# SYSTRAN/faster-whisper

Hardware: AMD Instinct MI355X
Metric: audio-sec/sec (RTF) large-v3 fp16 beam=5 batch=16 (higher is better)
Workload: dtype f16

## Files before the change

### faster_whisper_amd/_lib.py

```python
import ctypes as C
import os

import numpy as np

_HERE = os.path.dirname(os.path.abspath(__file__))
LIB_PATH = os.environ.get("FWAMD_LIB") or os.path.join(_HERE, "libfwamd.so")

FW_OK = 0
FW_EINVAL = -1
FW_ENODEV = -2
FW_ENOMEM = -3
FW_ERUNTIME = -4
FW_ENOSPC = -5

COMPUTE_FLOAT16 = 0
COMPUTE_INT8_FLOAT16 = 1
FW_DT_F32 = 0
FW_DT_F16 = 1
FW_MAX_ALIGN_HEADS = 64


class FwConfig(C.Structure):
    _fields_ = [
        ("n_mels", C.c_int32), ("n_audio_ctx", C.c_int32), ("d_model", C.c_int32), ("n_heads", C.c_int32),
# ... 40 lines not shown
    "fw_model_set_merge_wait", "fw_model_set_decode_lanes", "fw_model_run_capacity", "fw_dec_big_min_rows", "fw_dec_big_min_rows_of", "fw_test_knob",
    "fw_test_idle_lead_chunks",
    "fw_pack_blob_size", "fw_pack_blob_copy", "fw_pack_blob_free",
    "fw_logmel", "fw_logmel_full",
    "fw_encode", "fw_encode_pcm", "fw_encode_pcm_dev", "fw_tensor_shape", "fw_tensor_to_host",
    "fw_tensor_from_host", "fw_tensor_free",
    "fw_generate", "fw_generate_lp", "fw_detect_language", "fw_align",
    "fw_prof_enable", "fw_prof_reset", "fw_prof_count", "fw_prof_name", "fw_prof_get", "fw_synchronize",
    "fw_dev_alloc", "fw_dev_free", "fw_dev_upload",
    "fw_test_gemm", "fw_test_layernorm", "fw_test_attention", "fw_test_dec_linear", "fw_test_dec_logits", "fw_test_logits_rules",
    "fw_test_dec_self_attn", "fw_test_dec_cross_attn", "fw_test_dec_cross_probs", "fw_test_dec_softmax_pick", "fw_bench_gemm", "fw_bench_dec_linear", "fw_bench_attention",
    "fw_bench_gemm_epi", "fw_bench_dec_linear_epi",
    "fw_test_gemm_ex", "fw_test_cross_kv_frag_index", "fw_test_quant_rows", "fw_test_layernorm_frag",
    "fw_test_dec_beam_update", "fw_test_dec_embed", "fw_test_align_post",
    "fw_test_logits_rules_lp", "fw_test_dec_beam_update_lp",
    "fw_vad_create", "fw_vad_forward", "fw_vad_free", "fw_vad_forward_dev", "fw_vad_forward_audio_dev",
    "fw_vad_forward_audio_batch_dev",
    "fw_flac_info", "fw_flac_decode",
    "fw_resample_filter", "fw_resample_dev", "fw_bench_resample",
]

_lib = None


class FwError(RuntimeError):
    pass


def load():
    global _lib
# ... 70 lines not shown
    lib.fw_test_gemm.argtypes = [vp, vp, vp, vp, vp, i32, i32, i32, i32, i32, vp]
    lib.fw_test_dec_linear.argtypes = [vp, vp, vp, vp, vp, vp, vp, i32, i32, i32, i32, i32, vp, vp]
    lib.fw_test_dec_logits.argtypes = [vp, vp, i32, vp]
    lib.fw_test_logits_rules.argtypes = [vp, vp, i32, vp, i32, vp, C.POINTER(FwGenOpts), i32, vp, vp]
    if hasattr(lib, "fw_test_dec_self_attn"):
        lib.fw_test_dec_self_attn.argtypes = [vp, vp, vp, vp, vp, i32, i32, i32, i32, i32, i32, i32, i32, i32, i32, i32, vp]
        lib.fw_test_dec_cross_attn.argtypes = [vp, vp, vp, vp, i32, i32, i32, i32, i32, i32, vp, vp, i32, C.c_float, vp]
        lib.fw_test_dec_cross_probs.argtypes = [vp, vp, vp, i32, i32, i32, vp, i32, i32, i32, i32, vp]
        lib.fw_test_dec_softmax_pick.argtypes = [vp, vp, i32, i32, i32, vp, i32, vp]
    lib.fw_bench_attention.argtypes = [vp, i32, i32, i32, i32, i32, f32p]
    lib.fw_bench_gemm.argtypes = [vp, i32, i32, i32, i32, i32, i32, i32, i32, f32p]
    lib.fw_bench_dec_linear.argtypes = [vp, i32, i32, i32, i32, i32, i32, f32p]
    if hasattr(lib, "fw_bench_gemm_epi"):
        lib.fw_bench_gemm_epi.argtypes = [vp, i32, i32, i32, i32, i32, i32, i32, i32, i32, i32, i32, f32p]
        lib.fw_bench_dec_linear_epi.argtypes = [vp, i32, i32, i32, i32, i32, i32, i32, i32, i32, f32p]
    lib.fw_test_layernorm.argtypes = [vp, vp, vp, vp, i32, i32, vp]
    lib.fw_test_attention.argtypes = [vp, vp, vp, vp, i32, i32, i32, vp]
    if hasattr(lib, "fw_test_gemm_ex"):
        lib.fw_test_gemm_ex.argtypes = [vp, vp, i64, i64, i64, vp, vp, vp, i64, i64, i64, vp, i64, i64, i64, i64, i64,
                                        i32, i32, i32, i32, i32, i32, i32, i32, i32, vp, vp]
        lib.fw_test_cross_kv_frag_index.argtypes = [i32, i32, i32, vp]
        lib.fw_test_quant_rows.argtypes = [vp, vp, i32, i32, i64, vp, vp, i32, vp, vp]
        lib.fw_test_layernorm_frag.argtypes = [vp, vp, vp, vp, i32, i32, i32, vp]
    if hasattr(lib, "fw_test_dec_beam_update"):
        f32 = C.c_float
        lib.fw_test_dec_beam_update.argtypes = [vp, i32, i32, i32, i32, i32, i32, i32, i32, f32, i32, vp, vp, vp, vp, vp,
                                                i32, f32, vp, vp, vp, vp, vp, vp, vp, vp, vp, vp, vp]
        lib.fw_test_dec_embed.argtypes = [vp, vp, i32, vp, i32, vp, i32, i32, i32, i32, i32, i32, f32, vp, vp]
        lib.fw_test_align_post.argtypes = [vp, vp, i32, i32, i32, i32, vp, vp, i32, vp]
    if hasattr(lib, "fw_test_dec_beam_update_lp"):
# ... 46 lines not shown
```

### faster_whisper_amd/csrc/dec_kernels.h

```cpp
#pragma once
#include "common.h"

namespace fwd {

constexpr int FIN_CAP = 48;

struct GenDev {
  int B, K, R;
  int P;
  int budget;
  int max_fin;
  int V, n_text_ctx;
  int with_ts, suppress_blank, min_new, mits, ngram;
  float rep_pen, lp_pow;
  int eot, no_ts, ts_begin;
  int n_sup_begin, sup_begin[8];
  int sample;
  float inv_temp;
  unsigned seed_lo, seed_hi;
  int kv_div;
  int ctx, cache_rows;
  int ragged, reach;
};

// ... 22 lines not shown
                           int N, int K, int act);
int launch_dec_gemm_skinny_tiles(hipStream_t st, int tiles, const half_t* xf, const half_t* Wf, const half_t* bias,
                                 const float* s1, const float* cf, const half_t* res, int ldr, half_t* out, int ldo,
                                 half_t* out_frag, int R, int N, int K, int act);
int launch_dec_gemm_big(hipStream_t st, int cfg, const half_t* xf, const half_t* Wf, const half_t* bias, const float* s1,
                        const float* cf, const half_t* res, int ldr, half_t* out, int ldo, half_t* out_frag, int R,
                        int N, int K, int act);
int launch_dec_gemm_frag_variant(hipStream_t st, int variant, bool lnf, const half_t* xf, const half_t* Wf,
                                 const half_t* bias, const float* s1, const float* cf, half_t* out, int R, int N,
                                 int K);
int launch_dec_gemm_frag_i8(hipStream_t st, const int8_t* xq, const float* x_scale, const int8_t* Wq,
                            const float* w_scale, const half_t* bias, const half_t* res, int ldr, half_t* out, int ldo,
                            int R, int N, int K, int act);
int launch_dec_logits(hipStream_t st, bool i8, const void* xf, const float* x_scale, const void* Wf,
                      const float* w_scale, const float* s1, const float* cf, float* out, int ldo, int R, int N, int K);
void launch_nospeech(hipStream_t st, const float* logits, int V, int row_mul, int no_speech_id, float* out, int B);
#define LP_SUP_WORDS 896
void launch_logits_process(hipStream_t st, const GenDev& gp, float* logits, const unsigned long long* sup_bits,
                           const int* hist2, const float* cum2, const int* d_step, const int* done, float* cand_val,
                           int* cand_tok, float* cand_lp = nullptr);
void launch_beam_update(hipStream_t st, const GenDev& gp, const float* cand_val, const int* cand_tok, int* hist2,
                        float* cum2, uint8_t* kvidx2, int* cur_tok, const int* d_step, int* done, int* n_done,
                        int* n_fin, int* fin_tok, int* fin_len, float* fin_score, float* fin_cum,
                        const float* cand_lp = nullptr, float* lphist2 = nullptr, float* fin_lp = nullptr,
                        const int* ptab = nullptr);
void launch_gather_sot_rows(hipStream_t st, const half_t* x, const int* sot_tab, const int* ptab, int pos0, int nb,
                            int rows_per_chunk, half_t* xo, half_t* xof, int d, int B);
void launch_step_advance(hipStream_t st, int* d_step);
void launch_token_prob(hipStream_t st, const float* logits, int V, const int* target, float* out, int out_stride,
                       int out_off, int rows, int row_mul = 1);
// ... 5 lines not shown
```

### faster_whisper_amd/csrc/dec_kernels.hip

```cpp
#include "common.h"
#include "dec_kernels.h"
#include <stdlib.h>
#include <atomic>
#include <type_traits>

namespace fwd {
static std::atomic<int> g_self_attn_form{0};
static std::atomic<int> g_forms_epoch{0};
static std::atomic<int> g_cross_regs{0};
}

__device__ __forceinline__ size_t frag_off(int row, int k, int KS) {
  return ((size_t)((row >> 4) * KS + (k >> 5)) * 64 + ((k >> 3) & 3) * 16 + (row & 15)) * 8 + (k & 7);
}

static __device__ __forceinline__ int ragged_pos(const int* __restrict__ ptab, int chunk, int step, int reach) {
  const int p = ptab[chunk] - 1 + step;
  return p < reach ? p : reach - 1;
}

__global__ void dec_embed_kernel(const int* __restrict__ tok, const half_t* __restrict__ emb,
                                 const half_t* __restrict__ pos_emb, half_t* __restrict__ x,
                                 half_t* __restrict__ xfrag, int d, const int* __restrict__ d_step, int pos_fixed,
                                 int P, int blk_n, const int* __restrict__ ptab, int kmul, int reach) {
// ... 52 lines not shown
      const float t = tv - mu * a4[e];
      tv = rstd * t + c4[e];
    } else if (bias) {
      tv = tv + (float)b4[e];
    }
    if (act == 1) {
      const float er = erff(tv * 0.70710678118654752440f);
      tv = (0.5f * tv) * (1.0f + er);
    }
    if (has_res) tv = tv + (float)r4[e];
    o[e] = (half_t)tv;
  }
  return o;
}

static __device__ __forceinline__ half4_t dec_epilogue4_i8(const int (&v)[4], float sx, const float* __restrict__ w_scale,
                                                           const half_t* __restrict__ bias, const half_t* __restrict__ res,
                                                           int ldr, int row, int n, int act) {
#pragma clang fp contract(off)
  const floatx4 w4 = *reinterpret_cast<const floatx4*>(w_scale + n);
  half4_t b4 = {(half_t)0.f, (half_t)0.f, (half_t)0.f, (half_t)0.f}, r4 = b4;
  if (bias) b4 = *reinterpret_cast<const half4_t*>(bias + n);
  if (res) r4 = *reinterpret_cast<const half4_t*>(res + (size_t)row * ldr + n);
  half4_t o;
#pragma unroll
  for (int e = 0; e < 4; ++e) {
    float tv = ((float)v[e] * sx) * w4[e];
    if (bias) tv = tv + (float)b4[e];
    if (act == 1) {
      const float er = erff(tv * 0.70710678118654752440f);
// ... 160 lines not shown
#define DGB_TL_DECL
#endif
template <int N_>
static __device__ __forceinline__ void wait_vmcnt() {
  asm volatile("s_waitcnt vmcnt(%0)" ::"n"(N_) : "memory");
}
#define DGB_BARRIER()                      \
  do {                                     \
    asm volatile("" ::: "memory");         \
    __builtin_amdgcn_s_barrier();          \
    asm volatile("" ::: "memory");         \
  } while (0)

#define DGB_BARRIER_LDS() __syncthreads()

template <bool LNF, int S, int WM, int WN, int FB, int KC, int NST>
__global__ __launch_bounds__(WM * WN * 64, 2) void dec_gemm_big_kernel(
    const half_t* __restrict__ xf, const half_t* __restrict__ Wf, const half_t* __restrict__ bias,
    const float* __restrict__ s1, const float* __restrict__ cf, const half_t* __restrict__ res, int ldr,
    half_t* __restrict__ out, int ldo, half_t* __restrict__ out_frag, int R, int N, int K, int act, int nNt) {
  constexpr int NW = WM * WN;
  DGB_TL_DECL;
  constexpr int PX = 4 * WM, PW = FB * WN, PCS = PX + PW;
  static_assert((PCS * KC) % NW == 0, "pieces of a stage must divide over the waves");
  static_assert(FB == 2 || FB == 4, "column tiles per wave");
  constexpr int PPW = PCS * KC / NW;
  constexpr int STAGE_BYTES = PCS * KC * 1024;
  static_assert(NST >= 3 && NST <= 6, "ring depth");
  constexpr int DGB_EP_STRIDE = FB * 32 + 16;
  static_assert(NST * STAGE_BYTES >= NW * 64 * DGB_EP_STRIDE, "the epilogue stages one 64-row patch per wave through the ring");
  extern __shared__ __attribute__((aligned(16))) char dgb_smem[];
  const int lane = threadIdx.x & 63;
  const int wave = __builtin_amdgcn_readfirstlane(threadIdx.x >> 6);
  const int i = lane & 15, g = lane >> 4;
  const int wm = wave / WN, wn = wave % WN;
  const int bid = xcd_remap(blockIdx.x, gridDim.x);
  const int nMt = gridDim.x / nNt;
  const int nt = bid / nMt, mt = bid - nt * nMt;
  const int rt0 = mt * PX, ct0 = nt * PW;
  const int n_rt = (R + 15) >> 4;
  const int KS = K >> 5;
  const int per = KS / S;
  const int nch = KS / KC;
  const int ch_per_slice = per / KC;

  unsigned soff[PPW];
  const char* sbase[PPW];
#pragma unroll
  for (int q = 0; q < PPW; ++q) {
    const int p = wave * PPW + q;
    const int t = p / KC, ks = p % KC;
    if (t < PX) {
      int rt = rt0 + t;
      if (rt > n_rt - 1) rt = n_rt - 1;
      sbase[q] = reinterpret_cast<const char*>(xf);
      soff[q] = (unsigned)((((size_t)rt * KS + ks) * 64 + lane) * 16);
    } else {
      int ct = ct0 + t - PX;
      if (ct > (N >> 4) - 1) ct = (N >> 4) - 1;
      sbase[q] = reinterpret_cast<const char*>(Wf);
      soff[q] = (unsigned)((((size_t)ct * KS + ks) * 64 + lane) * 16);
    }
  }
  auto issue = [&](int c, int slot) {
    char* dst = dgb_smem + slot * STAGE_BYTES + wave * PPW * 1024;
    const unsigned koff = (unsigned)c * (KC * 1024);
#pragma unroll
    for (int q = 0; q < PPW; ++q)
      __builtin_amdgcn_global_load_lds((const __attribute__((address_space(1))) void*)(sbase[q] + (size_t)(soff[q] + koff)),
                                       (__attribute__((address_space(3))) void*)(dst + q * 1024), 16, 0, 0);
  };

  static_assert(!LNF || WN == 2, "the LayerNorm statistics are shared by the TWO waves of a row block");
  floatx4 acc[4][FB], tot[4][FB];
// ... 45 lines not shown
      }
    }
  };
  auto compute = [&](int slot) { fetch(slot); mma(); };
  auto slice_end = [&]() {
    if (LNF) {
#pragma unroll
      for (int aa = 0; aa < 2; ++aa) {
        float pa = rs[aa], pb = rq[aa];
        pa += __shfl_xor(pa, 16, 64); pa += __shfl_xor(pa, 32, 64);
        pb += __shfl_xor(pb, 16, 64); pb += __shfl_xor(pb, 32, 64);
        sal[aa] += pa; sbl[aa] += pb;
        rs[aa] = 0.f; rq[aa] = 0.f;
      }
    }
#pragma unroll
    for (int a = 0; a < 4; ++a) {
#pragma unroll
      for (int b = 0; b < FB; ++b) {
#pragma unroll
        for (int e = 0; e < 4; ++e) tot[a][b][e] += acc[a][b][e];
        acc[a][b] = floatx4{0, 0, 0, 0};
      }
    }
  };

#pragma unroll
  for (int c0 = 0; c0 < NST - 1; ++c0) issue(c0, c0);
  int slot = 0, fill = NST - 1;
  int to_slice = ch_per_slice;
// ... 12 lines not shown
    if (--to_slice == 0) { to_slice = ch_per_slice; slice_end(); }
    fill = slot;
    slot = (slot + 1 == NST) ? 0 : slot + 1;
  }
  wait_vmcnt<0>();
  const int row0 = (rt0 + wm * 4) * 16;
  const int col0 = (ct0 + wn * FB) * 16;
  constexpr int CPR = FB * 2;
  constexpr int RPI = 64 / CPR;
  const int cr = lane / CPR, cc = lane % CPR;
  constexpr int NSEG = 64 / RPI;
  constexpr int RES_EARLY = (LNF && NW == 8 && FB == 4) ? 2 : NSEG;
  DecColConsts colk[FB];
  intx4 resv[NSEG];
  auto load_res = [&](int j0, int j1) {
    if (!res) return;
#pragma unroll
    for (int j = 0; j < NSEG; ++j) {
      if (j < j0 || j >= j1) continue;
      int row = row0 + j * RPI + cr, n = col0 + cc * 8;
      if (row > R - 1) row = R - 1;
      if (n > N - 8) n = N - 8;
      resv[j] = *reinterpret_cast<const intx4*>(res + (size_t)row * ldr + n);
    }
  };
#pragma unroll
  for (int b = 0; b < FB; ++b) {
    int n = col0 + b * 16 + 4 * g;
    if (n > N - 4) n = N - 4;
    colk[b] = dec_col_consts<LNF>(s1, cf, bias, n);
  }
  load_res(0, RES_EARLY);
#pragma unroll 1
  for (int c = n_steady; c < nch; ++c) {
    DGB_BARRIER();
    compute(slot);
    if (--to_slice == 0) { to_slice = ch_per_slice; slice_end(); }
    slot = (slot + 1 == NST) ? 0 : slot + 1;
  }
  load_res(RES_EARLY, NSEG);
  DGB_BARRIER();

  if (LNF) {
// ... 1 lines not shown
    if (g == 0) {
#pragma unroll
      for (int aa = 0; aa < 2; ++aa) {
        xch[((wave * 2 + aa) * 16 + i) * 2] = sal[aa];
        xch[((wave * 2 + aa) * 16 + i) * 2 + 1] = sbl[aa];
      }
    }
    DGB_BARRIER_LDS();
#pragma unroll
    for (int a = 0; a < 4; ++a) {
      const int owner = (wave & ~1) | (a >> 1);
      sa[a] = xch[((owner * 2 + (a & 1)) * 16 + i) * 2];
      sb[a] = xch[((owner * 2 + (a & 1)) * 16 + i) * 2 + 1];
    }
    DGB_BARRIER_LDS();
  }
  char* ep = dgb_smem + wave * (64 * DGB_EP_STRIDE);
  if (res) {
#pragma unroll
    for (int j = 0; j < 64 / RPI; ++j) {
      const int r = j * RPI + cr;
      *reinterpret_cast<intx4*>(ep + r * DGB_EP_STRIDE + cc * 16) = resv[j];
    }
  }
#pragma unroll
  for (int a = 0; a < 4; ++a) {
    float mu = 0.f, rstd = 1.f;
    if (LNF) dec_ln_stats(sa[a], sb[a], K, mu, rstd);
#pragma unroll
    for (int b = 0; b < FB; ++b) {
// ... 1137 lines not shown
}

template <bool LNF, int RT, int NT, int CH = 0>
static void frag_go(hipStream_t st, int waves, const half_t* xf, const half_t* Wf, const half_t* bias, const float* s1,
                    const float* cf, const half_t* res, int ldr, half_t* out, int ldo, half_t* out_frag, int R, int N,
                    int K, int act) {
  const dim3 grid((N / 16 + NT - 1) / NT, ((R + 15) / 16 + RT - 1) / RT);
  if (waves == 8)
    dec_gemm_frag_kernel<8, LNF, RT, NT, CH><<<grid, 512, 0, st>>>(xf, Wf, bias, s1, cf, res, ldr, out, ldo, out_frag, R,
                                                                   N, K, act);
  else
    dec_gemm_frag_kernel<4, LNF, RT, NT, CH><<<grid, 256, 0, st>>>(xf, Wf, bias, s1, cf, res, ldr, out, ldo, out_frag, R,
                                                                   N, K, act);
}

template <bool LNF, int S, int WM, int WN, int FB, int KC, int NST>
static int big_go(hipStream_t st, const half_t* xf, const half_t* Wf, const half_t* bias, const float* s1, const float* cf,
                   const half_t* res, int ldr, half_t* out, int ldo, half_t* out_frag, int R, int N, int K, int act) {
  constexpr int lds = (4 * WM + FB * WN) * KC * 1024 * NST;
  static std::atomic<unsigned long long> attr_done{0};
  int dev = 0;
  (void)hipGetDevice(&dev);
  if (!((attr_done.load(std::memory_order_acquire) >> (dev & 63)) & 1ull)) {
    if (hipFuncSetAttribute(reinterpret_cast<const void*>(dec_gemm_big_kernel<LNF, S, WM, WN, FB, KC, NST>),
                            hipFuncAttributeMaxDynamicSharedMemorySize, lds) != hipSuccess)
      return -1;
    attr_done.fetch_or(1ull << (dev & 63), std::memory_order_release);
  }
  const int nMt = ((R + 15) / 16 + 4 * WM - 1) / (4 * WM), nNt = (N / 16 + FB * WN - 1) / (FB * WN);
  dec_gemm_big_kernel<LNF, S, WM, WN, FB, KC, NST><<<nMt * nNt, WM * WN * 64, lds, st>>>(xf, Wf, bias, s1, cf, res, ldr, out,
                                                                                           ldo, out_frag, R, N, K, act, nNt);
  return hipPeekAtLastError() == hipSuccess ? 0 : -1;
}
template <int WM, int WN, int FB, int KC, int NST>
static int big_cfg(hipStream_t st, const half_t* xf, const half_t* Wf, const half_t* bias, const float* s1, const float* cf,
                   const half_t* res, int ldr, half_t* out, int ldo, half_t* out_frag, int R, int N, int K, int act) {
  if (K % 32 != 0 || N % 32 != 0 || R < 1) return -1;
  const int S = K >= 2560 ? 8 : 4;
  const int KS = K / 32;
  if (KS % S != 0 || (KS / S) % KC != 0 || KS / KC < NST) return -1;
  if ((ldo % 8) || (res && (ldr % 8))) return -1;
#define DGB(LNF_, S_) big_go<LNF_, S_, WM, WN, FB, KC, NST>(st, xf, Wf, bias, s1, cf, res, ldr, out, ldo, out_frag, R, N, K, act)
  if (s1) return S == 8 ? DGB(true, 8) : DGB(true, 4);
  return S == 8 ? DGB(false, 8) : DGB(false, 4);
#undef DGB
}
int launch_dec_gemm_big(hipStream_t st, int cfg, const half_t* xf, const half_t* Wf, const half_t* bias, const float* s1,
// ... 43 lines not shown
      return launch_dec_gemm_big(st, variant - 10, xf, Wf, lnf ? nullptr : bias, lnf ? s1 : nullptr, lnf ? cf : nullptr,
                                 nullptr, 0, out, N, nullptr, R, N, K, 0);
    default: return -1;
  }
  return 0;
}

static int dec_linear_role(int N, int K) { return N == 3 * K ? 0 : (N >= 2560 ? 2 : (K >= 2560 ? 3 : 1)); }
struct DecBigRule { int rows; int cfg; };
static const DecBigRule DEC_BIG_RULES[4][2] = {
     {{640, 2}, {1280, 0}},
     {{1088, 1}, {1 << 30, 1}},
     {{512, 2}, {1280, 0}},
     {{832, 1}, {1 << 30, 1}},
};
static int dec_big_cfg_for(int R, int N, int K) {
  const DecBigRule* r = DEC_BIG_RULES[dec_linear_role(N, K)];
  if (R >= r[1].rows) return r[1].cfg;
  if (R >= r[0].rows) return r[0].cfg;
  return -1;
}
#define DEC_BIG_MIN_ROWS_I8 1024
int dec_big_min_rows_of(int role, int compute_type) {
  if (compute_type == 1) return DEC_BIG_MIN_ROWS_I8;
  if (role >= 0 && role < 4) return DEC_BIG_RULES[role][0].rows;
  int lo = DEC_BIG_RULES[0][0].rows;
  for (int k = 1; k < 4; ++k) lo = DEC_BIG_RULES[k][0].rows < lo ? DEC_BIG_RULES[k][0].rows : lo;
  return lo;
}

static bool skinny_one_tile(int R, int N) { return R <= 16 || (R <= 96 && N <= 1280); }

int launch_dec_gemm_frag(hipStream_t st, const half_t* xf, const half_t* Wf, const half_t* bias, const float* s1,
                         const float* cf, const half_t* res, int ldr, half_t* out, int ldo, half_t* out_frag, int R,
                         int N, int K, int act) {
  const int cfg = dec_big_cfg_for(R, N, K);
  if (cfg >= 0 &&
      launch_dec_gemm_big(st, cfg, xf, Wf, bias, s1, cf, res, ldr, out, ldo, out_frag, R, N, K, act) == 0)
// ... 55 lines not shown
    dec_gemm_frag_i8_kernel<4, 2, 2><<<grid, 256, 0, st>>>(xq, x_scale, Wq, w_scale, bias, res, ldr, out, ldo, R, N, K, act);
  return 0;
}

template <bool I8, bool LNF, int RT>
static void wave_go(hipStream_t st, const void* xf, const float* x_scale, const void* Wf, const float* w_scale,
                    const float* s1, const float* cf, float* out, int ldo, int R, int N, int K) {
  constexpr int NT = 2, WM = 1, WN = 4;
  const int n_rt = (R + 15) / 16, n_ct = (N + 15) / 16;
  const int n_cg = ((n_ct + NT * WN - 1) / (NT * WN) + 7) & ~7;
  const int n_rg = (n_rt + RT * WM - 1) / (RT * WM);
  dec_gemm_wave_kernel<I8, LNF, true, RT, NT, WM, WN><<<n_cg * n_rg, WM * WN * 64, 0, st>>>(
      xf, x_scale, Wf, w_scale, nullptr, s1, cf, out, ldo, R, N, K, n_rg);
}

int launch_dec_logits(hipStream_t st, bool i8, const void* xf, const float* x_scale, const void* Wf,
                      const float* w_scale, const float* s1, const float* cf, float* out, int ldo, int R, int N, int K) {
  if (K % (i8 ? 64 : 32) != 0 || R < 1) return -1;
  if (i8 ? (!x_scale || !w_scale) : ((s1 == nullptr) != (cf == nullptr))) return -1;
  const int n_rt = (R + 15) / 16;
#define WG(RT)                                                                                   \
  do {                                                                                           \
    if (i8) wave_go<true, false, RT>(st, xf, x_scale, Wf, w_scale, s1, cf, out, ldo, R, N, K);   \
    else if (s1) wave_go<false, true, RT>(st, xf, x_scale, Wf, w_scale, s1, cf, out, ldo, R, N, K); \
    else wave_go<false, false, RT>(st, xf, x_scale, Wf, w_scale, s1, cf, out, ldo, R, N, K);     \
  } while (0)
  if (n_rt == 1) WG(1);
  else if (n_rt == 2) WG(2);
  else if (n_rt == 3) WG(3);
  else if (n_rt == 4) WG(4);
  else WG(5);
#undef WG
  return 0;
}
// ... 117 lines not shown
```

### faster_whisper_amd/csrc/hooks.hip

```cpp
#include "engine.h"

#include <math.h>
#include <string.h>

#include <algorithm>

#include "dec_kernels.h"
#include "kernels.h"

using namespace fw;
using fwd::FIN_CAP;
using fwd::GenDev;

namespace {

struct HookBufs {
  std::vector<void*> p;
  HookBufs() = default;
  HookBufs(const HookBufs&) = delete;
  HookBufs& operator=(const HookBufs&) = delete;
  ~HookBufs() { for (void* q : p) (void)hipFree(q); }
  template <typename T>
  int alloc(T** dst, size_t n) {
    int rc = dev_alloc_t(dst, n);
// ... 243 lines not shown
      : use_int8 == 5 ? fwd::launch_dec_gemm_skinny(st, xfp, wfp, d_bias, d_s1, d_cf, d_res, N, d_out, N, d_of, R, N, K, act)
      : (use_int8 == 6 || use_int8 == 7) ? fwd::launch_dec_gemm_skinny_tiles(st, use_int8 - 5, xfp, wfp, d_bias, d_s1, d_cf, d_res, N, d_out, N, d_of, R, N, K, act)
                      : fwd::launch_dec_gemm_frag(st, xfp, wfp, d_bias, d_s1, d_cf, d_res, N, d_out, N, d_of, R, N, K, act);
  if (lr != 0) {
    set_error("decoder linear: unsupported shape R=%d N=%d K=%d", R, N, K);
    return FW_ERUNTIME;
  }
  if ((rc = download_f16(st, out, d_out, (size_t)R * N))) return rc;
  return download_f16_frag(st, out_from_frag, d_of, R, N);
}

int32_t fw_dec_big_min_rows(void) { return fwd::dec_big_min_rows(); }
int32_t fw_dec_big_min_rows_of(int32_t role, int32_t compute_type) { return fwd::dec_big_min_rows_of(role, compute_type); }

int32_t fw_test_knob(int32_t id, int32_t value) {
  FW_CHECK_ARG(id == 1 || id == 2 || id == 4 || id == 5 || id == 6 || id == 7, "unknown knob %d", id);
  if (id == 6) { set_cross_kv_layered(value); return FW_OK; }
  if (id == 7) { fwd::set_cross_attn_regs(value); return FW_OK; }
  if (id == 1) fwk::g_gemm_order.store(value);
  else if (id == 5) fwk::g_gemm_vt_stage.store(value);
  else if (id == 2) fwd::set_self_attn_form(value);
  else set_pos_blocks(value);
  return FW_OK;
}

int64_t fw_test_idle_lead_chunks(int64_t queued, int32_t n_queued, int32_t encoding, int64_t want, int32_t max_batch) {
  return idle_lead_chunks(queued, n_queued, encoding, want, max_batch);
}

int32_t fw_test_dec_logits(fw_model* fm, const float* x, int32_t R, float* out) {
  FW_CHECK_ARG(fm && x && out && R >= 1, "bad argument");
  Model* m = &fm->impl;
  std::lock_guard<std::mutex> lk(m->mu);
// ... 14 lines not shown
    float* d_xs;
    if ((rc = db.alloc(&d_xq, (size_t)R16 * d)) || (rc = db.alloc(&d_xs, (size_t)R16)) || (rc = db.zero(d_xq, (size_t)R16 * d, st)))
      return rc;
    fwk::launch_quant_rows(st, d_x, d, m->dec_ln.g, m->dec_ln.b, d_xq, d_xs, R, d, 1);
    lr = fwd::launch_dec_logits(st, true, d_xq, d_xs, m->logits.wq, m->logits.wscale, nullptr, nullptr, d_out, V, R, V, d);
  } else {
    lr = fwd::launch_dec_logits(st, false, d_x, nullptr, m->logits.w, nullptr, m->logits.s1, m->logits.cf, d_out, V, R, V,
                                d);
  }
  FW_HIP(hipStreamSynchronize(st));
  if (lr != 0) {
    set_error("logits projection test failed: unsupported shape");
    return FW_ERUNTIME;
  }
  return download(out, d_out, (size_t)R * V);
}

int32_t fw_bench_dec_linear(fw_model* fm, int32_t R, int32_t N, int32_t K, int32_t lnf, int32_t variant, int32_t iters,
                            float* us_out) {
  FW_CHECK_ARG(fm && us_out && R > 0 && N > 0 && K > 0 && iters > 0, "bad argument");
  Model* m = &fm->impl;
  std::lock_guard<std::mutex> lk(m->mu);
  FW_HIP(hipSetDevice(m->device));
  hipStream_t st = m->stream;
  const size_t wn = (size_t)N * K;
  const int copies = (int)std::max<size_t>(2, ((size_t)640 << 20) / (wn * 2));
  const size_t rp = ((size_t)R + 15) / 16 * 16;
  HookBufs db;
  half_t *dW, *dX, *dO, *dB;
  float *dS, *dC;
// ... 700 lines not shown
```

### profiles/dec_linear_bench.py

```python
import ctypes as C
import os
import sys

sys.path.insert(0, os.path.dirname(os.path.dirname(os.path.abspath(__file__))))
from faster_whisper_amd import Whisper, _lib, get_config, synthetic_weights

VARIANTS = {0: "4w 2x2 ch5 (product K<2560)", 1: "8w 2x2 ch5 (product K>=2560)", 2: "8w 4x2 ch3", 3: "8w 4x2 ch4",
            4: "8w 4x4 ch2", 5: "8w 4x4 ch3", 6: "4w 4x2 ch3", 7: "8w 2x4 ch3", 8: "8w 8x2 ch2", 9: "4w 4x4 ch2",
            10: "big 4x2 waves 256x128 KC2x3", 11: "big 2x2 waves 128x64 KC1x5", 12: "big 2x2 waves 128x128 KC1x4",
            13: "sp 4 slices x 2x2 waves 128x64 x3",
            21: "4w 4x4 ch5", 22: "8w 4x4 ch5", 23: "4w 1x1 ch10", 24: "8w 1x1 ch10", 25: "4w 1x2 ch6", 26: "8w 1x2 ch6"}
if os.environ.get("DLB_VARIANTS"):
    VARIANTS = {int(v): VARIANTS[int(v)] for v in os.environ["DLB_VARIANTS"].split(",")}
SHAPES = [("qkv", 3840, 1280, 1), ("dxd", 1280, 1280, 0), ("ffn1", 5120, 1280, 1), ("ffn2", 1280, 5120, 0)]
if os.environ.get("DLB_LNF") is not None:
    SHAPES = [(n, N, K, int(os.environ["DLB_LNF"])) for n, N, K, _ in SHAPES]

EPI_SHAPES = [("qkv", 3840, 1280, 1, 0, 0, 1), ("out", 1280, 1280, 0, 0, 1, 3), ("cross-q", 1280, 1280, 1, 0, 0, 1),
              ("cross-out", 1280, 1280, 0, 0, 1, 3), ("ffn1", 5120, 1280, 1, 1, 0, 2), ("ffn2", 1280, 5120, 0, 0, 1, 3)]


def epilogue_table(m, h, rows, reps=3, iters=400):
    us = C.c_float()
    for R in rows:
        print(f"R = {R}   us per launch, min .. max of {reps} measurements (bare = no activation / residual, row-major output only)")
        layer = {"bare": 0.0, "product": 0.0}
        for name, N, K, lnf, act, res, outs in EPI_SHAPES:
            t = {"bare": [], "product": []}
            for _ in range(reps):
                for key, (a_, r_, o_) in (("bare", (0, 0, 1)), ("product", (act, res, outs))):
                    _lib.check(m._lib.fw_bench_dec_linear_epi(h, R, N, K, lnf, 0, a_, r_, o_, iters, C.byref(us)))
                    t[key].append(us.value)
            for key in t:
                layer[key] += min(t[key])
            print("  %-10s bare %7.2f .. %7.2f   product %7.2f .. %7.2f" %
                  (name, min(t["bare"]), max(t["bare"]), min(t["product"]), max(t["product"])), flush=True)
        print("  %-10s bare %7.2f              product %7.2f" % ("layer", layer["bare"], layer["product"]), flush=True)


def main():
    cfg = get_config("micro")
    m = Whisper("synthetic:micro", device="cuda", files={"config": cfg, "weights": synthetic_weights(cfg, seed=1)},
                max_batch_size=1, max_beam_size=1)
    h = m._replicas[0].handle
    us = C.c_float()
    if "--epilogue" in sys.argv[1:]:
        epilogue_table(m, h, [int(a) for a in sys.argv[1:] if a != "--epilogue"] or [80, 800, 1280])
        return
    rows = [int(a) for a in sys.argv[1:]] or [80, 320, 640]
    for R in rows:
        print(f"R = {R}")
        print("  %-38s" % "variant" + "".join("%10s" % s[0] for s in SHAPES) + "   layer (qkv + 3 dxd + ffn1 + ffn2)   TFLOP/s")
        for v, name in VARIANTS.items():
            t = []
            for _, N, K, lnf in SHAPES:
                rc = m._lib.fw_bench_dec_linear(h, R, N, K, lnf, v, 400, C.byref(us))
                t.append(us.value if rc == 0 else float("nan"))
            layer = t[0] + 3 * t[1] + t[2] + t[3]
            flop = 2.0 * R * sum(n * k * (3 if nm == "dxd" else 1) for nm, n, k, _ in SHAPES)
            print("  %-38s" % name + "".join("%10.2f" % x for x in t) + "   %8.1f   %8.0f" % (layer, flop / layer / 1e6), flush=True)
# ... 5 lines not shown
```

Measured before the change: 3202.

## Route large-row fp16 vocabulary projection through the big GEMM kernel with fp32 epilogue

Adds a VP variant of the big decoder GEMM kernel that computes the vocabulary logits projection with folded LayerNorm, a ragged last column tile, and a float32 epilogue staged through LDS. launch_dec_logits now uses it by default for fp16 when there are at least 80 rows, and falls back to the wave-form kernel otherwise. The goal is better weight reuse and higher MFMA throughput on the large 51866x1280 logits GEMM at batch 16 with beam 5. It also adds a test knob, test and bench hooks, and a profiling table; the risks are numerical differences in the folded LN stats and out-of-bounds handling on the ragged edge.

```diff
diff --git a/faster_whisper_amd/_lib.py b/faster_whisper_amd/_lib.py
--- a/faster_whisper_amd/_lib.py
+++ b/faster_whisper_amd/_lib.py
@@ -78,6 +78,7 @@
     "fw_test_gemm_ex", "fw_test_cross_kv_frag_index", "fw_test_quant_rows", "fw_test_layernorm_frag",
     "fw_test_dec_beam_update", "fw_test_dec_embed", "fw_test_align_post",
     "fw_test_logits_rules_lp", "fw_test_dec_beam_update_lp",
+    "fw_test_logits_forms", "fw_bench_dec_logits",
     "fw_vad_create", "fw_vad_forward", "fw_vad_free", "fw_vad_forward_dev", "fw_vad_forward_audio_dev",
     "fw_vad_forward_audio_batch_dev",
     "fw_flac_info", "fw_flac_decode",
@@ -178,6 +179,9 @@
     if hasattr(lib, "fw_bench_gemm_epi"):
         lib.fw_bench_gemm_epi.argtypes = [vp, i32, i32, i32, i32, i32, i32, i32, i32, i32, i32, i32, f32p]
         lib.fw_bench_dec_linear_epi.argtypes = [vp, i32, i32, i32, i32, i32, i32, i32, i32, i32, f32p]
+    if hasattr(lib, "fw_test_logits_forms"):
+        lib.fw_test_logits_forms.argtypes = [vp, vp, vp, vp, vp, i32, i32, i32, i64, i32p, i32, vp, i64, i32p]
+        lib.fw_bench_dec_logits.argtypes = [vp, i32, i32, i32, i32p, i32, i32, i32, f32p]
     lib.fw_test_layernorm.argtypes = [vp, vp, vp, vp, i32, i32, vp]
     lib.fw_test_attention.argtypes = [vp, vp, vp, vp, i32, i32, i32, vp]
     if hasattr(lib, "fw_test_gemm_ex"):
diff --git a/faster_whisper_amd/csrc/dec_kernels.h b/faster_whisper_amd/csrc/dec_kernels.h
--- a/faster_whisper_amd/csrc/dec_kernels.h
+++ b/faster_whisper_amd/csrc/dec_kernels.h
@@ -60,6 +60,11 @@
                             int R, int N, int K, int act);
 int launch_dec_logits(hipStream_t st, bool i8, const void* xf, const float* x_scale, const void* Wf,
                       const float* w_scale, const float* s1, const float* cf, float* out, int ldo, int R, int N, int K);
+int launch_dec_logits_big(hipStream_t st, int cfg, const half_t* xf, const half_t* Wf, const float* s1, const float* cf,
+                          float* out, int ldo, int R, int N, int K);
+void set_logits_form(int form);
+int logits_form();
+int logits_last_form();
 void launch_nospeech(hipStream_t st, const float* logits, int V, int row_mul, int no_speech_id, float* out, int B);
 #define LP_SUP_WORDS 896
 void launch_logits_process(hipStream_t st, const GenDev& gp, float* logits, const unsigned long long* sup_bits,
diff --git a/faster_whisper_amd/csrc/dec_kernels.hip b/faster_whisper_amd/csrc/dec_kernels.hip
--- a/faster_whisper_amd/csrc/dec_kernels.hip
+++ b/faster_whisper_amd/csrc/dec_kernels.hip
@@ -90,6 +90,23 @@
   return o;
 }
 
+static __device__ __forceinline__ void logits_ln_stats(float sa, float sb, int K, float& mu, float& rstd) {
+#pragma clang fp contract(off)
+  const float kf = (float)K;
+  mu = sa / kf;
+  const float ex2 = sb / kf;
+  const float var = __builtin_fmaf(-mu, mu, ex2);
+  rstd = rsqrtf(fmaxf(var, 0.f) + 1e-5f);
+}
+static __device__ __forceinline__ floatx4 logits_epilogue4(const floatx4 v, float mu, float rstd, const floatx4 a4,
+                                                           const floatx4 c4) {
+#pragma clang fp contract(off)
+  floatx4 o;
+#pragma unroll
+  for (int e = 0; e < 4; ++e) o[e] = __builtin_fmaf(rstd, __builtin_fmaf(-mu, a4[e], v[e]), c4[e]);
+  return o;
+}
+
 static __device__ __forceinline__ half4_t dec_epilogue4_i8(const int (&v)[4], float sx, const float* __restrict__ w_scale,
                                                            const half_t* __restrict__ bias, const half_t* __restrict__ res,
                                                            int ldr, int row, int n, int act) {
@@ -280,7 +297,7 @@
 
 #define DGB_BARRIER_LDS() __syncthreads()
 
-template <bool LNF, int S, int WM, int WN, int FB, int KC, int NST>
+template <bool LNF, int S, int WM, int WN, int FB, int KC, int NST, bool VP = false>
 __global__ __launch_bounds__(WM * WN * 64, 2) void dec_gemm_big_kernel(
     const half_t* __restrict__ xf, const half_t* __restrict__ Wf, const half_t* __restrict__ bias,
     const float* __restrict__ s1, const float* __restrict__ cf, const half_t* __restrict__ res, int ldr,
@@ -295,6 +312,9 @@
   static_assert(NST >= 3 && NST <= 6, "ring depth");
   constexpr int DGB_EP_STRIDE = FB * 32 + 16;
   static_assert(NST * STAGE_BYTES >= NW * 64 * DGB_EP_STRIDE, "the epilogue stages one 64-row patch per wave through the ring");
+  constexpr int VP_EP_STRIDE = FB * 64 + 16;
+  static_assert(!VP || (LNF && S == 1), "the vocabulary projection: LayerNorm folded, one K slice");
+  static_assert(!VP || NST * STAGE_BYTES >= NW * 32 * VP_EP_STRIDE, "the float32 epilogue stages 32 rows per wave at a time");
   extern __shared__ __attribute__((aligned(16))) char dgb_smem[];
   const int lane = threadIdx.x & 63;
   const int wave = __builtin_amdgcn_readfirstlane(threadIdx.x >> 6);
@@ -323,7 +343,8 @@
       soff[q] = (unsigned)((((size_t)rt * KS + ks) * 64 + lane) * 16);
     } else {
       int ct = ct0 + t - PX;
-      if (ct > (N >> 4) - 1) ct = (N >> 4) - 1;
+      const int n_ct = VP ? (N + 15) >> 4 : N >> 4;
+      if (ct > n_ct - 1) ct = n_ct - 1;
       sbase[q] = reinterpret_cast<const char*>(Wf);
       soff[q] = (unsigned)((((size_t)ct * KS + ks) * 64 + lane) * 16);
     }
@@ -399,6 +420,7 @@
         rs[aa] = 0.f; rq[aa] = 0.f;
       }
     }
+    if (VP) return;
 #pragma unroll
     for (int a = 0; a < 4; ++a) {
 #pragma unroll
@@ -441,7 +463,7 @@
   DecColConsts colk[FB];
   intx4 resv[NSEG];
   auto load_res = [&](int j0, int j1) {
-    if (!res) return;
+    if (VP || !res) return;
 #pragma unroll
     for (int j = 0; j < NSEG; ++j) {
       if (j < j0 || j >= j1) continue;
@@ -454,6 +476,14 @@
 #pragma unroll
   for (int b = 0; b < FB; ++b) {
     int n = col0 + b * 16 + 4 * g;
+    if (VP) {
+#pragma unroll
+      for (int e = 0; e < 4; ++e) {
+        const int ne = n + e < N ? n + e : N - 1;
+        colk[b].a4[e] = s1[ne]; colk[b].c4[e] = cf[ne];
+      }
+      continue;
+    }
     if (n > N - 4) n = N - 4;
     colk[b] = dec_col_consts<LNF>(s1, cf, bias, n);
   }
@@ -485,6 +515,43 @@
       sb[a] = xch[((owner * 2 + (a & 1)) * 16 + i) * 2 + 1];
     }
     DGB_BARRIER_LDS();
+  }
+  if constexpr (VP) {
+    typedef float floatx4_a8 __attribute__((ext_vector_type(4), aligned(8)));
+    float* outf = reinterpret_cast<float*>(out);
+    char* epv = dgb_smem + wave * (32 * VP_EP_STRIDE);
+    constexpr int CPRV = FB * 4, RPIV = 64 / CPRV;
+    const int crv = lane / CPRV, ccv = lane % CPRV;
+    const bool vec_ok = (ldo & 1) == 0;
+#pragma unroll
+    for (int h = 0; h < 2; ++h) {
+#pragma unroll
+      for (int aa = 0; aa < 2; ++aa) {
+        const int a = 2 * h + aa;
+        float mu, rstd;
+        logits_ln_stats(sa[a], sb[a], K, mu, rstd);
+#pragma unroll
+        for (int b = 0; b < FB; ++b)
+          *reinterpret_cast<floatx4*>(epv + (aa * 16 + i) * VP_EP_STRIDE + (b * 16 + 4 * g) * 4) =
+              logits_epilogue4(acc[a][b], mu, rstd, colk[b].a4, colk[b].c4);
+      }
+#pragma unroll
+      for (int j = 0; j < 32 / RPIV; ++j) {
+        const int r = j * RPIV + crv;
+        const int row = row0 + h * 32 + r, n = col0 + ccv * 4;
+        const floatx4 v = *reinterpret_cast<const floatx4*>(epv + r * VP_EP_STRIDE + ccv * 16);
+        if (row >= R || n >= N) continue;
+        float* o = outf + (size_t)row * ldo + n;
+        if (vec_ok && n + 3 < N) {
+          *reinterpret_cast<floatx4_a8*>(o) = v;
+        } else {
+#pragma unroll
+          for (int e = 0; e < 4; ++e)
+            if (n + e < N) o[e] = v[e];
+        }
+      }
+    }
+    return;
   }
   char* ep = dgb_smem + wave * (64 * DGB_EP_STRIDE);
   if (res) {
@@ -1652,7 +1719,7 @@
                                                                    N, K, act);
 }
 
-template <bool LNF, int S, int WM, int WN, int FB, int KC, int NST>
+template <bool LNF, int S, int WM, int WN, int FB, int KC, int NST, bool VP = false>
 static int big_go(hipStream_t st, const half_t* xf, const half_t* Wf, const half_t* bias, const float* s1, const float* cf,
                    const half_t* res, int ldr, half_t* out, int ldo, half_t* out_frag, int R, int N, int K, int act) {
   constexpr int lds = (4 * WM + FB * WN) * KC * 1024 * NST;
@@ -1660,15 +1727,33 @@
   int dev = 0;
   (void)hipGetDevice(&dev);
   if (!((attr_done.load(std::memory_order_acquire) >> (dev & 63)) & 1ull)) {
-    if (hipFuncSetAttribute(reinterpret_cast<const void*>(dec_gemm_big_kernel<LNF, S, WM, WN, FB, KC, NST>),
+    if (hipFuncSetAttribute(reinterpret_cast<const void*>(dec_gemm_big_kernel<LNF, S, WM, WN, FB, KC, NST, VP>),
                             hipFuncAttributeMaxDynamicSharedMemorySize, lds) != hipSuccess)
       return -1;
     attr_done.fetch_or(1ull << (dev & 63), std::memory_order_release);
   }
-  const int nMt = ((R + 15) / 16 + 4 * WM - 1) / (4 * WM), nNt = (N / 16 + FB * WN - 1) / (FB * WN);
-  dec_gemm_big_kernel<LNF, S, WM, WN, FB, KC, NST><<<nMt * nNt, WM * WN * 64, lds, st>>>(xf, Wf, bias, s1, cf, res, ldr, out,
-                                                                                           ldo, out_frag, R, N, K, act, nNt);
+  const int n_ct = VP ? (N + 15) / 16 : N / 16;
+  const int nMt = ((R + 15) / 16 + 4 * WM - 1) / (4 * WM), nNt = (n_ct + FB * WN - 1) / (FB * WN);
+  dec_gemm_big_kernel<LNF, S, WM, WN, FB, KC, NST, VP><<<nMt * nNt, WM * WN * 64, lds, st>>>(xf, Wf, bias, s1, cf, res, ldr, out,
+                                                                                               ldo, out_frag, R, N, K, act, nNt);
   return hipPeekAtLastError() == hipSuccess ? 0 : -1;
+}
+template <int WM, int WN, int FB, int KC, int NST>
+static int logits_big_cfg(hipStream_t st, const half_t* xf, const half_t* Wf, const float* s1, const float* cf, float* out,
+                          int ldo, int R, int N, int K) {
+  if (K % 32 != 0 || R < 1 || N < 1 || !s1 || !cf) return -1;
+  const int KS = K / 32;
+  if (KS % KC != 0 || KS / KC < NST) return -1;
+  return big_go<true, 1, WM, WN, FB, KC, NST, true>(st, xf, Wf, nullptr, s1, cf, nullptr, 0, reinterpret_cast<half_t*>(out),
+                                                     ldo, nullptr, R, N, K, 0);
+}
+int launch_dec_logits_big(hipStream_t st, int cfg, const half_t* xf, const half_t* Wf, const float* s1, const float* cf,
+                          float* out, int ldo, int R, int N, int K) {
+  switch (cfg) {
+    case 0: return logits_big_cfg<4, 2, 4, 2, 3>(st, xf, Wf, s1, cf, out, ldo, R, N, K);
+    case 2: return logits_big_cfg<2, 2, 4, 1, 4>(st, xf, Wf, s1, cf, out, ldo, R, N, K);
+    default: return -1;
+  }
 }
 template <int WM, int WN, int FB, int KC, int NST>
 static int big_cfg(hipStream_t st, const half_t* xf, const half_t* Wf, const half_t* bias, const float* s1, const float* cf,
@@ -1742,6 +1827,7 @@
      {{512, 2}, {1280, 0}},
      {{832, 1}, {1 << 30, 1}},
 };
+static const DecBigRule DEC_LOGITS_BIG_RULE = {80, 2};
 static int dec_big_cfg_for(int R, int N, int K) {
   const DecBigRule* r = DEC_BIG_RULES[dec_linear_role(N, K)];
   if (R >= r[1].rows) return r[1].cfg;
@@ -1750,6 +1836,7 @@
 }
 #define DEC_BIG_MIN_ROWS_I8 1024
 int dec_big_min_rows_of(int role, int compute_type) {
+  if (role == 4) return compute_type == 1 ? 1 << 30 : DEC_LOGITS_BIG_RULE.rows;
   if (compute_type == 1) return DEC_BIG_MIN_ROWS_I8;
   if (role >= 0 && role < 4) return DEC_BIG_RULES[role][0].rows;
   int lo = DEC_BIG_RULES[0][0].rows;
@@ -1835,10 +1922,26 @@
       xf, x_scale, Wf, w_scale, nullptr, s1, cf, out, ldo, R, N, K, n_rg);
 }
 
+static std::atomic<int> g_logits_form{0};
+static std::atomic<int> g_logits_last_form{0};
+void set_logits_form(int form) { g_logits_form.store(form); g_forms_epoch.fetch_add(1); }
+int logits_form() { return g_logits_form.load(); }
+int logits_last_form() { return g_logits_last_form.load(); }
+
 int launch_dec_logits(hipStream_t st, bool i8, const void* xf, const float* x_scale, const void* Wf,
                       const float* w_scale, const float* s1, const float* cf, float* out, int ldo, int R, int N, int K) {
   if (K % (i8 ? 64 : 32) != 0 || R < 1) return -1;
   if (i8 ? (!x_scale || !w_scale) : ((s1 == nullptr) != (cf == nullptr))) return -1;
+  if (!i8 && s1) {
+    const int forced = g_logits_form.load();
+    const int cfg = forced == 2 ? 2 : forced == 3 ? 0 : (forced == 0 && R >= DEC_LOGITS_BIG_RULE.rows) ? DEC_LOGITS_BIG_RULE.cfg : -1;
+    if (cfg >= 0 && launch_dec_logits_big(st, cfg, reinterpret_cast<const half_t*>(xf), reinterpret_cast<const half_t*>(Wf),
+                                          s1, cf, out, ldo, R, N, K) == 0) {
+      g_logits_last_form.store(cfg == 2 ? 2 : 3);
+      return 0;
+    }
+  }
+  g_logits_last_form.store(1);
   const int n_rt = (R + 15) / 16;
 #define WG(RT)                                                                                   \
   do {                                                                                           \
diff --git a/faster_whisper_amd/csrc/hooks.hip b/faster_whisper_amd/csrc/hooks.hip
--- a/faster_whisper_amd/csrc/hooks.hip
+++ b/faster_whisper_amd/csrc/hooks.hip
@@ -281,9 +281,14 @@
 int32_t fw_dec_big_min_rows_of(int32_t role, int32_t compute_type) { return fwd::dec_big_min_rows_of(role, compute_type); }
 
 int32_t fw_test_knob(int32_t id, int32_t value) {
-  FW_CHECK_ARG(id == 1 || id == 2 || id == 4 || id == 5 || id == 6 || id == 7, "unknown knob %d", id);
+  FW_CHECK_ARG(id == 1 || id == 2 || id == 4 || id == 5 || id == 6 || id == 7 || id == 8, "unknown knob %d", id);
   if (id == 6) { set_cross_kv_layered(value); return FW_OK; }
   if (id == 7) { fwd::set_cross_attn_regs(value); return FW_OK; }
+  if (id == 8) {
+    FW_CHECK_ARG(value >= 0 && value <= 3, "knob 8: 0 by row count, 1 wave form, 2 / 3 GEMM-shaped form");
+    fwd::set_logits_form(value);
+    return FW_OK;
+  }
   if (id == 1) fwk::g_gemm_order.store(value);
   else if (id == 5) fwk::g_gemm_vt_stage.store(value);
   else if (id == 2) fwd::set_self_attn_form(value);
@@ -328,6 +333,84 @@
     return FW_ERUNTIME;
   }
   return download(out, d_out, (size_t)R * V);
+}
+
+int32_t fw_test_logits_forms(fw_model* fm, const float* x, const float* W, const float* s1, const float* cf, int32_t R,
+                             int32_t N, int32_t K, int64_t ldo, const int32_t* forms, int32_t n_forms, float* out,
+                             int64_t out_elems, int32_t* taken) {
+  FW_CHECK_ARG(fm && x && W && s1 && cf && forms && out && taken, "null argument");
+  FW_CHECK_ARG(R >= 1 && N >= 1 && K >= 32 && K % 32 == 0 && n_forms >= 1, "need R >= 1, N >= 1, K %% 32 == 0, n_forms >= 1");
+  FW_CHECK_ARG(ldo >= N && ldo < ((int64_t)1 << 31) && (int64_t)(R - 1) * ldo + N <= out_elems, "out [out_elems] does not hold R rows of stride ldo");
+  for (int f = 0; f < n_forms; ++f) FW_CHECK_ARG(forms[f] >= 0 && forms[f] <= 3, "form %d", forms[f]);
+  Model* m = &fm->impl;
+  std::lock_guard<std::mutex> lk(m->mu);
+  FW_HIP(hipSetDevice(m->device));
+  hipStream_t st = m->stream;
+  const int64_t R16 = ((int64_t)R + 15) / 16 * 16, N16 = ((int64_t)N + 15) / 16 * 16;
+  std::vector<uint16_t> xh((size_t)(R16 * K), 0), wh((size_t)(N16 * K), 0);
+  for (int64_t r = 0; r < R; ++r)
+    for (int64_t k = 0; k < K; ++k) xh[frag_pos(r, k, K, 32)] = f32_to_f16_bits(x[r * K + k]);
+  for (int64_t n = 0; n < N; ++n)
+    for (int64_t k = 0; k < K; ++k) wh[frag_pos(n, k, K, 32)] = f32_to_f16_bits(W[n * K + k]);
+  HookBufs db;
+  uint16_t *d_x, *d_w;
+  float *d_s1, *d_cf, *d_out;
+  int rc;
+  if ((rc = db.upload(&d_x, xh.data(), xh.size())) || (rc = db.upload(&d_w, wh.data(), wh.size())) ||
+      (rc = db.upload(&d_s1, s1, (size_t)N)) || (rc = db.upload(&d_cf, cf, (size_t)N)) || (rc = db.alloc(&d_out, (size_t)out_elems)))
+    return rc;
+  const int before = fwd::logits_form();
+  int lr = 0;
+  for (int f = 0; f < n_forms && lr == 0 && rc == 0; ++f) {
+    float* o = out + (size_t)f * out_elems;
+    FW_HIP(hipMemcpyAsync(d_out, o, (size_t)out_elems * 4, hipMemcpyHostToDevice, st));
+    fwd::set_logits_form(forms[f]);
+    lr = fwd::launch_dec_logits(st, false, d_x, nullptr, d_w, nullptr, d_s1, d_cf, d_out, (int)ldo, R, N, K);
+    taken[f] = fwd::logits_last_form();
+    fwd::set_logits_form(before);
+    if (hipStreamSynchronize(st) != hipSuccess) { set_error("logits forms: the launch failed"); return FW_ERUNTIME; }
+    if (lr == 0) rc = download(o, d_out, (size_t)out_elems);
+  }
+  if (lr != 0) { set_error("logits forms: unsupported shape R=%d N=%d K=%d", R, N, K); return FW_ERUNTIME; }
+  return rc;
+}
+
+int32_t fw_bench_dec_logits(fw_model* fm, int32_t R, int32_t N, int32_t K, const int32_t* forms, int32_t n_forms,
+                            int32_t reps, int32_t iters, float* us_out) {
+  FW_CHECK_ARG(fm && us_out && forms && R > 0 && N > 0 && K > 0 && K % 32 == 0 && iters > 0 && n_forms > 0 && reps > 0, "bad argument");
+  for (int f = 0; f < n_forms; ++f) FW_CHECK_ARG(forms[f] >= 0 && forms[f] <= 3, "form %d", forms[f]);
+  Model* m = &fm->impl;
+  std::lock_guard<std::mutex> lk(m->mu);
+  FW_HIP(hipSetDevice(m->device));
+  hipStream_t st = m->stream;
+  const size_t wn = ((size_t)N + 15) / 16 * 16 * K, xn = ((size_t)R + 15) / 16 * 16 * K;
+  const int wcopies = (int)std::max<size_t>(2, ((size_t)512 << 20) / (wn * 2) + 1);
+  const int xcopies = (int)std::max<size_t>(2, ((size_t)288 << 20) / (xn * 2) + 1);
+  HookBufs db;
+  half_t *dW, *dX;
+  float *dS, *dC, *dO;
+  std::vector<uint16_t> stage;
+  int rc;
+  if ((rc = db.alloc(&dW, wn * wcopies)) || (rc = db.alloc(&dX, xn * xcopies)) || (rc = db.alloc(&dO, (size_t)R * N)) ||
+      (rc = db.alloc(&dS, (size_t)N)) || (rc = db.alloc(&dC, (size_t)N)) ||
+      (rc = fill_lcg(dW, wn, stage, 2463534242u, 1e-3f)) || (rc = fill_lcg(dX, xn, stage, 88172645u, 1e-3f)) ||
+      (rc = db.zero(dS, (size_t)N * 4, st)) || (rc = db.zero(dC, (size_t)N * 4, st)))
+    return rc;
+  for (int c = 1; c < wcopies; ++c) FW_HIP(hipMemcpy(dW + (size_t)c * wn, dW, wn * 2, hipMemcpyDeviceToDevice));
+  for (int c = 1; c < xcopies; ++c) FW_HIP(hipMemcpy(dX + (size_t)c * xn, dX, xn * 2, hipMemcpyDeviceToDevice));
+  const int before = fwd::logits_form();
+  for (int q = 0; q < reps * n_forms && rc == 0; ++q) {
+    fwd::set_logits_form(forms[q % n_forms]);
+    float ms = 0.f;
+    rc = time_launches(st, 2, iters, [&](int i) {
+      return fwd::launch_dec_logits(st, false, dX + (size_t)(i % xcopies) * xn, nullptr, dW + (size_t)(i % wcopies) * wn, nullptr,
+                                    dS, dC, dO, N, R, N, K);
+    }, &ms);
+    us_out[q] = ms * 1000.f / (float)iters;
+  }
+  fwd::set_logits_form(before);
+  if (rc == LAUNCH_REFUSED) { set_error("fw_bench_dec_logits: unsupported shape"); return FW_EINVAL; }
+  return rc;
 }
 
 int32_t fw_bench_dec_linear(fw_model* fm, int32_t R, int32_t N, int32_t K, int32_t lnf, int32_t variant, int32_t iters,
diff --git a/profiles/dec_linear_bench.py b/profiles/dec_linear_bench.py
--- a/profiles/dec_linear_bench.py
+++ b/profiles/dec_linear_bench.py
@@ -38,12 +38,33 @@
         print("  %-10s bare %7.2f              product %7.2f" % ("layer", layer["bare"], layer["product"]), flush=True)
 
 
+LOGITS_FORMS = {1: "wave 80x128", 2: "big 128x128", 3: "big 256x128", 0: "product"}
+LOGITS_ROWS = [80, 160, 320, 480, 640, 800, 1040, 1280, 1600]
+
+
+def logits_table(m, h, rows, N=51866, K=1280, reps=3, iters=24):
+    forms = list(LOGITS_FORMS)
+    print(f"logits {N} x {K}: us per launch, min .. max of {reps} alternating measurements of {iters} launches; "
+          f"product rule: GEMM-shaped from {m._lib.fw_dec_big_min_rows_of(4, 0)} rows")
+    print("  %6s" % "rows" + "".join("%24s" % LOGITS_FORMS[f] for f in forms) + "   TFLOP/s (best)")
+    for R in rows:
+        us = (C.c_float * (reps * len(forms)))()
+        _lib.check(m._lib.fw_bench_dec_logits(h, R, N, K, (C.c_int32 * len(forms))(*forms), len(forms), reps, iters, us))
+        t = [[us[r * len(forms) + k] for r in range(reps)] for k in range(len(forms))]
+        best = min(min(x) for x in t)
+        print("  %6d" % R + "".join("%12.1f ..%9.1f" % (min(x), max(x)) for x in t) + "   %8.0f" % (2.0 * R * N * K / best / 1e6),
+              flush=True)
+
+
 def main():
     cfg = get_config("micro")
     m = Whisper("synthetic:micro", device="cuda", files={"config": cfg, "weights": synthetic_weights(cfg, seed=1)},
                 max_batch_size=1, max_beam_size=1)
     h = m._replicas[0].handle
     us = C.c_float()
+    if "logits" in sys.argv[1:]:
+        logits_table(m, h, [int(a) for a in sys.argv[1:] if a != "logits"] or LOGITS_ROWS)
+        return
     if "--epilogue" in sys.argv[1:]:
         epilogue_table(m, h, [int(a) for a in sys.argv[1:] if a != "--epilogue"] or [80, 800, 1280])
         return
```

New measurement: 3199. Within noise of the previous version (-0.1%).
